# ForJadeForest/DistillCLIP

Measured on AMD Instinct MI355X. Metric: image-text pairs/sec (distill step), higher is better.
Workload: dtype bf16; 1 GPU; l_clip.yaml dual distill: ViT-B/32 CLIP teacher -> weight-shared ViT(6x768,24h,R2) + text(4x768,12h,R2) students, 224px/77tok, losses out_l1+out_cos+0.1*cos_diff, fwd+loss+bwd+AdamW; global_batch=512, batch_per_gpu=512, parallelism=dp1, gradient_exchange=none, negatives=local (reference training_step semantics), optimizer_in_step=True, teacher_residual=fp16, saved_gelu_derivative=u8 fixed point, clock_probe=True

## Files before the change

distillclip_amd/csrc/gemm.hip:

```cpp

#include "gemm_common.h"
#include <atomic>

using namespace dgemm;

namespace {

constexpr int TILE_BYTES = (BM / 16) * (BK / 32) * SUB;
constexpr int CLD = BN + 4;
constexpr int NT_LDS = (4 * TILE_BYTES > BM * CLD * 4) ? 4 * TILE_BYTES : BM * CLD * 4;


__device__ __forceinline__ void stage_operand(const bf16_t* __restrict__ G, int64_t ld, int row0, int rows_max,
                                              int k0, char* lds_tile, int wave, int lane) {
    const int L = lane * 16;
    const int X = swz(L);
    const int r = X >> 6, c = (X >> 4) & 3;
#pragma unroll
    for (int s = 0; s < 4; ++s) {
        const int sub = wave * 4 + s;
        const int rb = sub >> 1, kb = sub & 1;
        int row = row0 + rb * 16 + r;
        row = row < rows_max ? row : rows_max - 1;
        const bf16_t* src = G + (int64_t)row * ld + (k0 + kb * 32 + c * 8);
        __builtin_amdgcn_global_load_lds((gbl_void*)src, (lds_void*)(lds_tile + sub * SUB), 16, 0, 0);
    }
}

template <int ACT, int OUT>
__global__ __launch_bounds__(256) void gemm_nt_kernel(GemmNT p) {
    extern __shared__ __attribute__((aligned(16))) char smem[];
    const int tid = threadIdx.x, lane = tid & 63;
    const int wave = __builtin_amdgcn_readfirstlane(tid >> 6);
    const int wm = wave >> 1, wn = wave & 1;

    const int nwg = p.tiles_m * p.tiles_n;
    const int t = xcd_remap(blockIdx.x, nwg);
    const int tm = t / p.tiles_n, tn = t % p.tiles_n;
    const int m0 = tm * BM, n0 = tn * BN;

    char* As = smem;
    char* Bs = smem + 2 * TILE_BYTES;

    f32x4 acc[4][4];
#pragma unroll
    for (int i = 0; i < 4; ++i)
#pragma unroll
        for (int j = 0; j < 4; ++j) acc[i][j] = f32x4{0.f, 0.f, 0.f, 0.f};

    const int nk = p.K / BK;
    stage_operand(p.A, p.lda, m0, p.M, 0, As, wave, lane);
    stage_operand(p.B, p.ldb, n0, p.N, 0, Bs, wave, lane);

    const int fragoff = swz((lane & 15) * 64 + (lane >> 4) * 16);

    for (int kt = 0; kt < nk; ++kt) {
        __syncthreads();
        if (kt + 1 < nk) {
            const int nb = (kt + 1) & 1;
            stage_operand(p.A, p.lda, m0, p.M, (kt + 1) * BK, As + nb * TILE_BYTES, wave, lane);
            stage_operand(p.B, p.ldb, n0, p.N, (kt + 1) * BK, Bs + nb * TILE_BYTES, wave, lane);
        }
        const char* a_t = As + (kt & 1) * TILE_BYTES;
        const char* b_t = Bs + (kt & 1) * TILE_BYTES;
#pragma unroll
        for (int kb = 0; kb < 2; ++kb) {
            bf16x8 af[4], bfr[4];
#pragma unroll
            for (int i = 0; i < 4; ++i)
                af[i] = *(const bf16x8*)(a_t + ((wm * 4 + i) * 2 + kb) * SUB + fragoff);
#pragma unroll
            for (int j = 0; j < 4; ++j)
                bfr[j] = *(const bf16x8*)(b_t + ((wn * 4 + j) * 2 + kb) * SUB + fragoff);
#pragma unroll
            for (int i = 0; i < 4; ++i)
#pragma unroll
                for (int j = 0; j < 4; ++j)
                    acc[i][j] = __builtin_amdgcn_mfma_f32_16x16x32_bf16(af[i], bfr[j], acc[i][j], 0, 0, 0);
        }
    }

    __syncthreads();
    float* cs = (float*)smem;
#pragma unroll
    for (int i = 0; i < 4; ++i)
#pragma unroll
        for (int j = 0; j < 4; ++j)
#pragma unroll
            for (int r = 0; r < 4; ++r)
                cs[(wm * 64 + i * 16 + (lane >> 4) * 4 + r) * CLD + wn * 64 + j * 16 + (lane & 15)] = acc[i][j][r];
    __syncthreads();
    const int cc = (tid & 15) * 8;
    const int col = n0 + cc;
    const bool col_ok = col < p.N;
    float bias[8];
#pragma unroll
    for (int e = 0; e < 8; ++e) bias[e] = 0.f;
    if (p.bias && col_ok) {
        const float4 b0 = *(const float4*)(p.bias + col), b1 = *(const float4*)(p.bias + col + 4);
        bias[0] = b0.x; bias[1] = b0.y; bias[2] = b0.z; bias[3] = b0.w; bias[4] = b1.x; bias[5] = b1.y; bias[6] = b1.z; bias[7] = b1.w;
    }
    float csum[8];
#pragma unroll
    for (int e = 0; e < 8; ++e) csum[e] = 0.f;
#pragma unroll
    for (int it = 0; it < 8; ++it) {
        const int rl = (tid >> 4) + it * 16;
        const int row = m0 + rl;
        if (row >= p.M || !col_ok) break;
        float v[8];
        {
            const float4 c0 = *(const float4*)(cs + rl * CLD + cc), c1 = *(const float4*)(cs + rl * CLD + cc + 4);
            v[0] = c0.x; v[1] = c0.y; v[2] = c0.z; v[3] = c0.w; v[4] = c1.x; v[5] = c1.y; v[6] = c1.z; v[7] = c1.w;
        }
#pragma unroll
        for (int e = 0; e < 8; ++e) v[e] = v[e] * p.alpha + bias[e];
        if (p.row_group > 0) {
            const float* ra = p.rowadd + (int64_t)(row % p.row_group) * p.N + col;
            const float4 a0 = *(const float4*)ra, a1 = *(const float4*)(ra + 4);
            v[0] += a0.x; v[1] += a0.y; v[2] += a0.z; v[3] += a0.w; v[4] += a1.x; v[5] += a1.y; v[6] += a1.z; v[7] += a1.w;
        }
        const int64_t o = (int64_t)row * p.ldc + col;
        {
            EpiSide sd;
            epilogue_load_side<ACT, OUT>(p, o, (int64_t)row * p.ldr + col, sd);
            float zero[8] = {0.f, 0.f, 0.f, 0.f, 0.f, 0.f, 0.f, 0.f}, unused[8];
            GemmNT q = p;
            q.alpha = 1.f; q.row_group = 0; q.colsum = nullptr;
            epilogue_vec8<ACT, OUT, 0>(q, v, row, col, o, (int64_t)row * p.ldr + col, zero, unused, sd);
        }
#pragma unroll
        for (int e = 0; e < 8; ++e) csum[e] += v[e];
    }
    if (p.colsum) {
        __syncthreads();
#pragma unroll
        for (int e = 0; e < 8; ++e) cs[(tid >> 4) * CLD + cc + e] = csum[e];
        __syncthreads();
        if (tid < BN && n0 + tid < p.N) {
            float x = 0.f;
#pragma unroll
            for (int r = 0; r < 16; ++r) x += cs[r * CLD + tid];
            unsafeAtomicAdd(p.colsum + n0 + tid, x);
        }
    }
}

constexpr int HT = 16384;

__device__ __forceinline__ void stage_half_perm(const bf16_t* __restrict__ G, int64_t ld, int row0, int rows_max, int k0,
                                                char* buf, int wave, int lane) {
    const int L = lane * 16;
    const int X = swz(L);
    const int r = X >> 6, c = (X >> 4) & 3;
    const int j = wave & 3;
    int row = row0 + (wave >> 2) * 64 + (j >> 1) * 32 + (r >> 2) * 8 + (j & 1) * 4 + (r & 3);
    row = row < rows_max ? row : rows_max - 1;
    const bf16_t* src = G + (int64_t)row * ld + k0 + c * 8;
    __builtin_amdgcn_global_load_lds((gbl_void*)src, (lds_void*)(buf + (wave * 2 + 0) * SUB), 16, 0, 0);
    __builtin_amdgcn_global_load_lds((gbl_void*)(src + 32), (lds_void*)(buf + (wave * 2 + 1) * SUB), 16, 0, 0);
}

template <int RH>
__device__ __forceinline__ void stage_rowhalf(const bf16_t* __restrict__ G, int64_t ld, int m0, int rows_max, int k0,
                                              char* abase, int hta, int dn, int wave, int lane) {
    const int L = lane * 16;
    const int X = swz(L);
    const int r = X >> 6, c = (X >> 4) & 3;
    constexpr int AROWS = RH * 32;
    {
        const int wv = RH == 3 ? wave % 6 : wave;
        const int g = wv / RH, i = wv % RH + dn * RH;
        int row = m0 + g * AROWS + i * 16 + r;
        row = row < rows_max ? row : rows_max - 1;
        const bf16_t* src = G + (int64_t)row * ld + k0 + c * 8;
        char* dst = abase + g * hta + (i * 2) * SUB;
        __builtin_amdgcn_global_load_lds((gbl_void*)src, (lds_void*)dst, 16, 0, 0);
        __builtin_amdgcn_global_load_lds((gbl_void*)(src + 32), (lds_void*)(dst + SUB), 16, 0, 0);
    }
    if (RH == 5) {
        const int e = wave & 3, rbk = 8 + (e >> 1), kb = e & 1;
        const int g = rbk / RH, i = rbk % RH + dn * RH;
        int row = m0 + g * AROWS + i * 16 + r;
        row = row < rows_max ? row : rows_max - 1;
        const bf16_t* src = G + (int64_t)row * ld + k0 + kb * 32 + c * 8;
        __builtin_amdgcn_global_load_lds((gbl_void*)src, (lds_void*)(abase + g * hta + (i * 2 + kb) * SUB), 16, 0, 0);
    }
}


__device__ __forceinline__ float row16_sum(float x) {
    auto dpp = [](float v, auto ctrl) {
        return __builtin_bit_cast(float, __builtin_amdgcn_update_dpp(0, __builtin_bit_cast(int, v), decltype(ctrl)::value, 0xf, 0xf, false));
    };
    x += dpp(x, std::integral_constant<int, 0xB1>{});
    x += dpp(x, std::integral_constant<int, 0x4E>{});
    x += dpp(x, std::integral_constant<int, 0x141>{});
    x += dpp(x, std::integral_constant<int, 0x140>{});
    return x;
}

template <int ACT, int OUT, int MI>
__global__ __launch_bounds__(512) void gemm_nt256_kernel(GemmNT p) {
    extern __shared__ __attribute__((aligned(16))) char smem[];
    constexpr int RH = MI / 2;
    constexpr int AROWS = MI * 16;
    constexpr int HTA = AROWS * BK * 2;
    constexpr int PAR = 2 * HT + 2 * HTA;
    constexpr int BMT = 2 * AROWS;
    const int tid = threadIdx.x, lane = tid & 63;
    const int wave = __builtin_amdgcn_readfirstlane(tid >> 6);
    const int wr = wave >> 2, wc = wave & 3;

    const int nwg = p.tiles_m * p.tiles_n;
    const int nk = p.K / BK;
    const int nload = 4 * nk;
    int m0, n0;
    auto locate = [&](int tl) {
        const int t = xcd_remap(tl, nwg);
        int tm, tn;
        if (p.group_n >= p.tiles_n) { tm = t / p.tiles_n; tn = t % p.tiles_n; }
        else {
            const int per = p.tiles_m * p.group_n;
            const int gi = t / per, rem = t - gi * per;
            const int left = p.tiles_n - gi * p.group_n;
            const int gw = left < p.group_n ? left : p.group_n;
            tm = rem / gw; tn = gi * p.group_n + rem % gw;
        }
        m0 = tm * BMT; n0 = tn * 256;
    };
    locate(blockIdx.x);

    f32x4 acc[MI][4];

    const int ln = lane;
    auto issue = [&](int l) {
        const int tile = l >> 2, w = l & 3;
        char* par = smem + (tile & 1) * PAR;
        if (w < 2) stage_half_perm(p.B, p.ldb, n0 + w * 128, p.N, tile * BK, par + w * HT, wave, ln);
        else stage_rowhalf<RH>(p.A, p.lda, m0, p.M, tile * BK, par + 2 * HT, HTA, w - 2, wave, ln);
    };
    auto stamp = [&](int k) {
        if (p.stamps && tid == 0) {
            if (k == 3) WAIT_VMCNT(0);
            p.stamps[6 * (int64_t)blockIdx.x + k] = __builtin_readcyclecounter();
            if (k == 0) p.stamps[6 * (int64_t)blockIdx.x + 4] = __builtin_amdgcn_s_memrealtime();
            if (k == 3) p.stamps[6 * (int64_t)blockIdx.x + 5] = __builtin_amdgcn_s_memrealtime();
        }
    };
    stamp(0);
    if (p.clk && blockIdx.x == 0 && tid == 0) { p.clk[0] = __builtin_amdgcn_s_memtime(); p.clk[1] = __builtin_amdgcn_s_memrealtime(); }
#define WAIT_VM2(n8, n10) do { if (MI == 10) WAIT_VMCNT(n10); else WAIT_VMCNT(n8); } while (0)
    const int npro = nload < 7 ? nload : 7;
    for (int l = 0; l < npro; ++l) issue(l);
    const int a_off = 2 * HT + wr * HTA;
    const int b_off = (wc >> 1) * HT + (wc & 1) * 8 * SUB;
    const int fragoff = swz((ln & 15) * 64 + (ln >> 4) * 16);
#pragma unroll
    for (int i = 0; i < MI; ++i)
#pragma unroll
        for (int j = 0; j < 4; ++j) acc[i][j] = f32x4{0.f, 0.f, 0.f, 0.f};
    if (nload > 4) WAIT_VM2(8, 10); else WAIT_VMCNT(0);
    __builtin_amdgcn_s_barrier();
    stamp(1);
    if (wr == 1) __builtin_amdgcn_s_barrier();

    bf16x8 af[RH][2], b0[2][2], b1[2][2];

    for (int kt = 0; kt < nk; ++kt) {
        const char* base = smem + (kt & 1) * PAR;
        const char* ap = base + a_off + fragoff;
        const char* bp = base + b_off + fragoff;
#pragma unroll
        for (int j = 0; j < 2; ++j)
#pragma unroll
            for (int kb = 0; kb < 2; ++kb) {
                b0[j][kb] = *(const bf16x8*)(bp + (j * 2 + kb) * SUB);
                b1[j][kb] = *(const bf16x8*)(bp + ((2 + j) * 2 + kb) * SUB);
            }
        __builtin_amdgcn_sched_barrier(0);
#pragma unroll
        for (int i = 0; i < RH; ++i)
#pragma unroll
            for (int kb = 0; kb < 2; ++kb) af[i][kb] = *(const bf16x8*)(ap + (i * 2 + kb) * SUB);
        if (kt + 1 < nk) { issue(4 * (kt + 1) + 3); WAIT_VM2(8, 10); }
        else WAIT_VMCNT(0);
        WAIT_LGKM0();
        __builtin_amdgcn_s_barrier();
        __builtin_amdgcn_s_setprio(1);
#pragma unroll
        for (int kb = 0; kb < 2; ++kb)
#pragma unroll
            for (int i = 0; i < RH; ++i) {
#pragma unroll
                for (int j = 0; j < 2; ++j)
                    acc[i][j] = __builtin_amdgcn_mfma_f32_16x16x32_bf16(b0[j][kb], af[i][kb], acc[i][j], 0, 0, 0);
#pragma unroll
                for (int j = 0; j < 2; ++j)
                    acc[i][2 + j] = __builtin_amdgcn_mfma_f32_16x16x32_bf16(b1[j][kb], af[i][kb], acc[i][2 + j], 0, 0, 0);
            }
        __builtin_amdgcn_s_setprio(0);
        __builtin_amdgcn_s_barrier();
#pragma unroll
        for (int i = 0; i < RH; ++i)
#pragma unroll
            for (int kb = 0; kb < 2; ++kb) af[i][kb] = *(const bf16x8*)(ap + ((RH + i) * 2 + kb) * SUB);
        if (kt + 2 < nk) { issue(4 * (kt + 2)); issue(4 * (kt + 2) + 1); issue(4 * (kt + 2) + 2); WAIT_VM2(8, 10); }
        else if (kt + 1 < nk) WAIT_VM2(2, 3);
        else WAIT_VMCNT(0);
        WAIT_LGKM0();
        __builtin_amdgcn_s_barrier();
        __builtin_amdgcn_s_setprio(1);
#pragma unroll
        for (int kb = 0; kb < 2; ++kb)
#pragma unroll
            for (int i = 0; i < RH; ++i) {
#pragma unroll
                for (int j = 0; j < 2; ++j)
                    acc[RH + i][j] = __builtin_amdgcn_mfma_f32_16x16x32_bf16(b0[j][kb], af[i][kb], acc[RH + i][j], 0, 0, 0);
#pragma unroll
                for (int j = 0; j < 2; ++j)
                    acc[RH + i][2 + j] = __builtin_amdgcn_mfma_f32_16x16x32_bf16(b1[j][kb], af[i][kb], acc[RH + i][2 + j], 0, 0, 0);
            }
        __builtin_amdgcn_s_setprio(0);
        __builtin_amdgcn_s_barrier();
    }
    if (wr == 0) __builtin_amdgcn_s_barrier();
    stamp(2);
    const int m0c = m0, n0c = n0;
    const int g = ln >> 4, rl = ln & 15;

    const int colb = n0c + wc * 64 + g * 8;
    float bias[2][8], csum[2][8];
#pragma unroll
    for (int jp = 0; jp < 2; ++jp) {
#pragma unroll
        for (int e = 0; e < 8; ++e) { bias[jp][e] = 0.f; csum[jp][e] = 0.f; }
        const int col = colb + jp * 32;
        if (p.bias && col < p.N) {
            const float4 q0 = *(const float4*)(p.bias + col), q1 = *(const float4*)(p.bias + col + 4);
            bias[jp][0] = q0.x; bias[jp][1] = q0.y; bias[jp][2] = q0.z; bias[jp][3] = q0.w;
            bias[jp][4] = q1.x; bias[jp][5] = q1.y; bias[jp][6] = q1.z; bias[jp][7] = q1.w;
        }
    }
    constexpr bool OUT_F32 = OUT == 1;
    constexpr bool SIDE = OUT != 0 || ACT == 3 || ACT == 4;
    constexpr int NU = 2 * MI;
    constexpr int BU = !SIDE ? NU : (OUT_F32 ? ((ACT == 3 || ACT == 4) ? 4 : (MI == 8 ? 8 : (MI == 6 ? 6 : 5))) : (MI == 10 ? 10 : NU));
    static_assert(NU % BU == 0, "batch size must divide the unit count");
    EpiSide side[SIDE ? BU : 1];
    const int row0 = m0c + wr * AROWS + rl;
    const int64_t o0 = (int64_t)row0 * p.ldc + colb, r0off = (int64_t)row0 * p.ldr + colb;
    const int64_t ostep = 16 * p.ldc, rstep = 16 * p.ldr;
    const bool full = m0c + BMT <= p.M && n0c + 256 <= p.N;
    auto run_units = [&](auto mode_tag) {
        constexpr int MODE = decltype(mode_tag)::value;
#pragma unroll
        for (int ub = 0; ub < NU; ub += BU) {
            if (SIDE) {
#pragma unroll
                for (int u = ub; u < ub + BU; ++u) {
                    const int i = u >> 1, jp = u & 1;
                    if (full || (row0 + i * 16 < p.M && colb + jp * 32 < p.N))
                        epilogue_load_side<ACT, OUT>(p, o0 + i * ostep + jp * 32, r0off + i * rstep + jp * 32, side[u - ub]);
                }
            }
#pragma unroll
            for (int u = ub; u < ub + BU; ++u) {
                const int i = u >> 1, jp = u & 1;
                const int row = row0 + i * 16, col = colb + jp * 32;
                if (full || (row < p.M && col < p.N)) {
                    float v[8];
#pragma unroll
                    for (int r = 0; r < 4; ++r) { v[r] = acc[i][2 * jp][r]; v[4 + r] = acc[i][2 * jp + 1][r]; }
                    epilogue_vec8<ACT, OUT, MODE>(p, v, row, col, o0 + i * ostep + jp * 32, r0off + i * rstep + jp * 32, bias[jp], csum[jp],
                                                      side[SIDE ? u - ub : 0]);
                }
            }
        }
    };
    const bool lean = p.row_group == 0 && ((ACT == 5 || ACT == 6) ? p.aux_out != nullptr : p.aux_out == nullptr) && (OUT != 0 ? p.residual != nullptr : p.residual == nullptr);
    if constexpr (OUT != 0) {
        if (lean) run_units(std::integral_constant<int, 3>{});
        else run_units(std::integral_constant<int, 0>{});
    } else if constexpr (ACT == 3 || ACT == 4) {
        if (lean && p.colsum) run_units(std::integral_constant<int, 2>{});
        else run_units(std::integral_constant<int, 0>{});
    } else {
        if (lean && !p.colsum) run_units(std::integral_constant<int, 1>{});
        else if (lean) run_units(std::integral_constant<int, 2>{});
        else run_units(std::integral_constant<int, 0>{});
    }
    if (OUT == 0 && p.colsum) {
        float* cs = (float*)smem;
#pragma unroll
        for (int jp = 0; jp < 2; ++jp)
#pragma unroll
            for (int e = 0; e < 8; ++e) {
                const float x = row16_sum(csum[jp][e]);
                if (rl == 0) cs[wr * 256 + wc * 64 + jp * 32 + g * 8 + e] = x;
            }
        WAIT_LGKM0();
        __builtin_amdgcn_s_barrier();
        const int tc = wave * 64 + ln;
        if (tc < 256 && n0c + tc < p.N) unsafeAtomicAdd(p.colsum + n0c + tc, cs[tc] + cs[256 + tc]);
    }
    stamp(3);
    if (p.clk && blockIdx.x == 0 && tid == 0) { p.clk[2] = __builtin_amdgcn_s_memtime(); p.clk[3] = __builtin_amdgcn_s_memrealtime(); }
}

constexpr int TP = 128, TQ = 128, TC = 64;
constexpr int TROW = 288;
constexpr int TTILE = TC * TROW;

struct GemmTN {
    const bf16_t* A; int64_t lda;
    const bf16_t* B; int64_t ldb;
    float* out; int64_t ldo;
    int M, P, Q;
    int tiles_p, tiles_q, splits, chunk;
    unsigned long long* stamps;
    float* partial;
};

__device__ __forceinline__ void tn_load(const bf16_t* __restrict__ G, int64_t ld, int m0, int m_end, int c0, int cols,
                                        int tid, u32x4 (&regs)[4]) {
#pragma unroll
    for (int s = 0; s < 4; ++s) {
        const int idx = s * 256 + tid;
        const int r = idx >> 4, c = (idx & 15) * 8;
        const int row = m0 + r, col = c0 + c;
        if (row < m_end && col < cols) regs[s] = *(const u32x4*)(G + (int64_t)row * ld + col);
        else regs[s] = u32x4{0u, 0u, 0u, 0u};
    }
}
__device__ __forceinline__ void tn_store(char* tile, int tid, const u32x4 (&regs)[4]) {
#pragma unroll
    for (int s = 0; s < 4; ++s) {
        const int idx = s * 256 + tid;
        const int r = idx >> 4, c = (idx & 15);
        *(u32x4*)(tile + r * TROW + c * 16) = regs[s];
    }
}

typedef __attribute__((address_space(3))) s16x4 lds_s16x4;

__device__ __forceinline__ bf16x8 tr_frag(const char* tile, int r0, int x0, int lane) {
    const int g = lane >> 4, q = (lane >> 2) & 3, pp = lane & 3;
// ... 225 lines not shown
    const int tid = threadIdx.x, lane = tid & 63;
    const int wave = __builtin_amdgcn_readfirstlane(tid >> 6);
    const int wr = wave >> 2, wc = wave & 3;

    const int tiles = p.tiles_p * p.tiles_q;
    const int t = xcd_remap(blockIdx.x, tiles * p.splits);
    const int split = t / tiles, tile = t - split * tiles;
    const int tq = tile % p.tiles_q, tp = tile / p.tiles_q;
    const int p0 = tp * 256, q0 = tq * 256;
    const int m_begin = split * p.chunk;
    const int m_end = min(p.M, m_begin + p.chunk);
    if (m_begin >= m_end) return;
    const int nk = (m_end - m_begin) / TC;
    const int nload = 4 * nk;

    f32x4 acc[8][4];
#pragma unroll
    for (int i = 0; i < 8; ++i)
#pragma unroll
        for (int j = 0; j < 4; ++j) acc[i][j] = f32x4{0.f, 0.f, 0.f, 0.f};

    const char* srcs[4][2];
    tn_half_sources(p.B, p.ldb, m_begin, q0, wave, lane, srcs[0]);
    tn_half_sources(p.B, p.ldb, m_begin, q0 + 128, wave, lane, srcs[1]);
    tn_half_sources(p.A, p.lda, m_begin, p0, wave, lane, srcs[2]);
    tn_half_sources(p.A, p.lda, m_begin, p0 + 128, wave, lane, srcs[3]);
    const int64_t step_b = (int64_t)TC * p.ldb * 2, step_a = (int64_t)TC * p.lda * 2;
    auto issue = [&](int l) {
        const int kt = l >> 2, w = l & 3;
        char* buf = smem + ((kt & 1) * 4 + w) * HT;
        if (w == 0) stage_half_tn(srcs[0], kt * step_b, buf, wave);
        else if (w == 1) stage_half_tn(srcs[1], kt * step_b, buf, wave);
        else if (w == 2) stage_half_tn(srcs[2], kt * step_a, buf, wave);
        else stage_half_tn(srcs[3], kt * step_a, buf, wave);
    };
    auto stamp = [&](int k) {
        if (p.stamps && tid == 0) {
            if (k == 3) WAIT_VMCNT(0);
            p.stamps[6 * (int64_t)blockIdx.x + k] = __builtin_readcyclecounter();
            if (k == 0) p.stamps[6 * (int64_t)blockIdx.x + 4] = __builtin_amdgcn_s_memrealtime();
            if (k == 3) p.stamps[6 * (int64_t)blockIdx.x + 5] = __builtin_amdgcn_s_memrealtime();
        }
    };
    stamp(0);
    const int npro = nload < 6 ? nload : 6;
#pragma unroll
    for (int l = 0; l < 6; ++l)
        if (l < npro) issue(l);
    if (nload > 4) WAIT_VMCNT(4); else WAIT_VMCNT(0);
    __builtin_amdgcn_s_barrier();
    stamp(1);
    if (wr == 1) __builtin_amdgcn_s_barrier();

    const int a_off = (2 + wr) * HT;
    const int b_off = (wc >> 1) * HT;
    const int bcol = (wc & 1) * 64;
    bf16x8 af[4][2], b0[2][2], b1[2][2];

    for (int kt = 0; kt < nk; ++kt) {
        const char* base = smem + (kt & 1) * 4 * HT;
        const char* at = base + a_off;
        const char* bt = base + b_off;
        const int k4 = kt * 4;
#pragma unroll
        for (int j = 0; j < 2; ++j) {
            const unsigned a0 = tr_frag_base(bt, bcol + j * 16, lane), a1 = tr_frag_base(bt, bcol + (2 + j) * 16, lane);
            b0[j][0] = tr_frag_asm<0>(a0); b0[j][1] = tr_frag_asm<32 * 256>(a0);
            b1[j][0] = tr_frag_asm<0>(a1); b1[j][1] = tr_frag_asm<32 * 256>(a1);
        }
        __builtin_amdgcn_sched_barrier(0);
#pragma unroll
        for (int i = 0; i < 4; ++i) {
            const unsigned a0 = tr_frag_base(at, i * 16, lane);
            af[i][0] = tr_frag_asm<0>(a0); af[i][1] = tr_frag_asm<32 * 256>(a0);
        }
        if (k4 + 6 < nload) issue(k4 + 6);
        if (k4 + 7 < nload) issue(k4 + 7);
        WAIT_LGKM0();
        __builtin_amdgcn_sched_barrier(0);
        __builtin_amdgcn_s_barrier();
        __builtin_amdgcn_s_setprio(1);
#pragma unroll
        for (int kb = 0; kb < 2; ++kb)
#pragma unroll
            for (int i = 0; i < 4; ++i) {
#pragma unroll
                for (int j = 0; j < 2; ++j)
                    acc[i][j] = __builtin_amdgcn_mfma_f32_16x16x32_bf16(af[i][kb], b0[j][kb], acc[i][j], 0, 0, 0);
#pragma unroll
                for (int j = 0; j < 2; ++j)
                    acc[i][2 + j] = __builtin_amdgcn_mfma_f32_16x16x32_bf16(af[i][kb], b1[j][kb], acc[i][2 + j], 0, 0, 0);
            }
        __builtin_amdgcn_s_setprio(0);
        __builtin_amdgcn_s_barrier();
        __builtin_amdgcn_sched_barrier(0);
#pragma unroll
        for (int i = 0; i < 4; ++i) {
            const unsigned a0 = tr_frag_base(at, (4 + i) * 16, lane);
            af[i][0] = tr_frag_asm<0>(a0); af[i][1] = tr_frag_asm<32 * 256>(a0);
        }
        if (k4 + 8 < nload) { issue(k4 + 8); issue(k4 + 9); WAIT_VMCNT(4); }
        else WAIT_VMCNT(0);
        WAIT_LGKM0();
        __builtin_amdgcn_sched_barrier(0);
        __builtin_amdgcn_s_barrier();
        __builtin_amdgcn_s_setprio(1);
#pragma unroll
        for (int kb = 0; kb < 2; ++kb)
#pragma unroll
            for (int i = 0; i < 4; ++i) {
#pragma unroll
                for (int j = 0; j < 2; ++j)
                    acc[4 + i][j] = __builtin_amdgcn_mfma_f32_16x16x32_bf16(af[i][kb], b0[j][kb], acc[4 + i][j], 0, 0, 0);
#pragma unroll
                for (int j = 0; j < 2; ++j)
                    acc[4 + i][2 + j] = __builtin_amdgcn_mfma_f32_16x16x32_bf16(af[i][kb], b1[j][kb], acc[4 + i][2 + j], 0, 0, 0);
            }
        __builtin_amdgcn_s_setprio(0);
        __builtin_amdgcn_s_barrier();
    }
    if (wr == 0) __builtin_amdgcn_s_barrier();
    stamp(2);

    float* cs = (float*)smem;
    constexpr int CL = 256 + 4;
#pragma unroll
    for (int q = 0; q < 4; ++q) {
        __syncthreads();
#pragma unroll
        for (int i = 0; i < 2; ++i)
#pragma unroll
            for (int j = 0; j < 4; ++j)
#pragma unroll
                for (int r = 0; r < 4; ++r)
                    cs[(wr * 32 + i * 16 + (lane >> 4) * 4 + r) * CL + wc * 64 + j * 16 + (lane & 15)] = acc[q * 2 + i][j][r];
        __syncthreads();
        if (p.partial) {
            float* dst = p.partial + ((int64_t)split * tiles + tile) * 65536;
#pragma unroll 4
            for (int it = 0; it < 8; ++it) {
                const int sl = (tid >> 6) + it * 8;
                const int rt = (sl >> 5) * 128 + q * 32 + (sl & 31);
                *(float4*)(dst + rt * 256 + (tid & 63) * 4) = *(const float4*)&cs[sl * CL + (tid & 63) * 4];
            }
        } else {
#pragma unroll 4
            for (int it = 0; it < 32; ++it) {
                const int sl = (tid >> 8) + it * 2;
                const int row = p0 + (sl >> 5) * 128 + q * 32 + (sl & 31);
                const int col = q0 + (tid & 255);
                unsafeAtomicAdd(p.out + (int64_t)row * p.ldo + col, cs[sl * CL + (tid & 255)]);
            }
        }
    }
    stamp(3);
}

__global__ __launch_bounds__(256) void tn256_reduce_kernel(const float* __restrict__ partial, int splits, int tiles, int tiles_q,
                                                           float* __restrict__ out, int64_t ldo) {
    const int idx = blockIdx.x * 256 + threadIdx.x;
    const int tile = idx >> 14, rt = (idx >> 6) & 255, c4 = idx & 63;
    if (tile >= tiles) return;
    const float* src = partial + (int64_t)tile * 65536 + rt * 256 + c4 * 4;
    float4 a = *(const float4*)src;
    for (int s = 1; s < splits; ++s) {
        const float4 v = *(const float4*)(src + (int64_t)s * tiles * 65536);
        a.x += v.x; a.y += v.y; a.z += v.z; a.w += v.w;
    }
    float* o = out + (int64_t)((tile / tiles_q) * 256 + rt) * ldo + (tile % tiles_q) * 256 + c4 * 4;
    float4 cur = *(const float4*)o;
    cur.x += a.x; cur.y += a.y; cur.z += a.z; cur.w += a.w;
    *(float4*)o = cur;
}

__global__ __launch_bounds__(256) void colsum_kernel(const bf16_t* __restrict__ X, int64_t ld, float* __restrict__ db,
                                                     int M, int N, int rows_per_block) {
    const int col = blockIdx.x * 256 + threadIdx.x;
    if (col >= N) return;
    const int r0 = blockIdx.y * rows_per_block;
    const int r1 = min(M, r0 + rows_per_block);
    float s0 = 0.f, s1 = 0.f, s2 = 0.f, s3 = 0.f;
    int r = r0;
    for (; r + 3 < r1; r += 4) {
        s0 += bf2f(X[(int64_t)r * ld + col]);
        s1 += bf2f(X[(int64_t)(r + 1) * ld + col]);
        s2 += bf2f(X[(int64_t)(r + 2) * ld + col]);
        s3 += bf2f(X[(int64_t)(r + 3) * ld + col]);
    }
    for (; r < r1; ++r) s0 += bf2f(X[(int64_t)r * ld + col]);
    unsafeAtomicAdd(db + col, (s0 + s1) + (s2 + s3));
}

__global__ __launch_bounds__(256) void colsum8_kernel(const bf16_t* __restrict__ X, int64_t ld, float* __restrict__ db,
                                                      int M, int N, int rows_per_block) {
    __shared__ float red[8][256 + 8];
    const int cg = threadIdx.x & 31, rl = threadIdx.x >> 5;
    const int col = blockIdx.x * 256 + cg * 8;
    const int r0 = blockIdx.y * rows_per_block;
    const int r1 = min(M, r0 + rows_per_block);
    float acc[8];
#pragma unroll
    for (int e = 0; e < 8; ++e) acc[e] = 0.f;
    if (col < N) {
        int r = r0 + rl;
        for (; r + 24 < r1; r += 32) {
            bf16x8 v[4];
#pragma unroll
            for (int u = 0; u < 4; ++u) v[u] = *(const bf16x8*)(X + (int64_t)(r + 8 * u) * ld + col);
#pragma unroll
            for (int u = 0; u < 4; ++u)
#pragma unroll
                for (int e = 0; e < 8; ++e) acc[e] += bf2f(v[u][e]);
        }
        for (; r < r1; r += 8) {
            const bf16x8 v = *(const bf16x8*)(X + (int64_t)r * ld + col);
#pragma unroll
            for (int e = 0; e < 8; ++e) acc[e] += bf2f(v[e]);
        }
    }
#pragma unroll
    for (int e = 0; e < 8; ++e) red[rl][cg * 8 + e] = acc[e];
    __syncthreads();
    const int c = blockIdx.x * 256 + threadIdx.x;
    if (c < N) {
        float x = 0.f;
#pragma unroll
        for (int w = 0; w < 8; ++w) x += red[w][threadIdx.x];
        unsafeAtomicAdd(db + c, x);
    }
}

bool use_256(const GemmNT& p) {
    static const int mode = [] { const char* e = getenv("DCLIP_GEMM256"); return e ? atoi(e) : 1; }();
    return mode != 0 && p.M >= 1024 && p.N >= 256;
}

std::atomic<unsigned long long*> g_clock_buf{nullptr};
std::atomic<long long> g_clock_cap{0};
std::atomic<long long> g_clock_count{0};
inline unsigned long long* next_clock_slot() {
    unsigned long long* buf = g_clock_buf.load(std::memory_order_acquire);
    const long long cap = g_clock_cap.load(std::memory_order_relaxed);
    if (!buf || cap <= 0) return nullptr;
    return buf + 4 * (g_clock_count.fetch_add(1, std::memory_order_relaxed) % cap);
}

template <int ACT>
int launch_nt(GemmNT p, int out, hipStream_t st) {
    if constexpr (ACT != 0) { if (out == 2) { dclip_set_error("dclip_gemm_nt: f16 output needs act = DCLIP_ACT_NONE"); return DCLIP_EINVAL; } }
    const bool out_f32 = out == 1;
    if (use_256(p) && !(out != 0 && p.colsum) && (ACT == 0 || out == 0)) {
        int tm = (p.M + 255) / 256;
        const int tn = (p.N + 255) / 256;
        static const int mode320 = [] { const char* e = getenv("DCLIP_GEMM320"); return e ? atoi(e) : 1; }();
        int mi = 8;
        if (mode320) {
            const double nkt = (double)(p.K / BK), e8 = out_f32 ? 40000.0 : out == 2 ? 24000.0 : (ACT == 0 || ACT == 4 ? 9500.0 : 14000.0);
            auto cost = [&](int rows, double per_kt, double escale) {
                const int tmx = (p.M + rows - 1) / rows;
                return (double)((tmx * tn + 255) / 256) * (3300.0 + nkt * per_kt + escale * e8);
            };
            const double c8 = cost(256, 2750.0, 1.0), c10 = cost(320, 3200.0, 1.25), c6 = cost(192, 2150.0, 0.75);
            if (mode320 == 2) mi = 10;
            else if (mode320 == 6) mi = 6;
            else {
                if (c10 < c8) mi = 10;
                if (c6 < (mi == 10 ? c10 : c8) * 0.97) mi = 6;
            }
            tm = (p.M + mi * 32 - 1) / (mi * 32);
        }
        p.tiles_m = tm; p.tiles_n = tn;
        p.clk = next_clock_slot();
        const int ntiles = p.tiles_m * p.tiles_n;
        {
            const double panel = 512.0 * (double)p.K, a_bytes = 2.0 * (double)p.M * (double)p.K;
            double best = 0.0; int best_g = tn;
            for (int g = 1; g <= tn; ++g) {
                const int ngroups = (tn + g - 1) / g;
                const double b_term = (g * panel <= 2.5e6) ? 8.0 * g * panel * (ngroups > 8 ? ngroups / 8.0 : 1.0)
                                                           : (double)ntiles / 32.0 * g * panel;
                const double cost = a_bytes * ngroups + b_term;
                if (g == 1 || cost < best * 0.999) { best = cost; best_g = g; }
            }
            p.group_n = best_g;
        }
        if (mi == 10) {
            const size_t lds320 = 2 * (2 * HT + 2 * 160 * BK * 2) + 16;
            if (out_f32) { if constexpr (ACT == 0) hipLaunchKernelGGL((gemm_nt256_kernel<0, 1, 10>), dim3(ntiles), dim3(512), lds320, st, p); }
            else if (out == 2) { if constexpr (ACT == 0) hipLaunchKernelGGL((gemm_nt256_kernel<0, 2, 10>), dim3(ntiles), dim3(512), lds320, st, p); }
            else hipLaunchKernelGGL((gemm_nt256_kernel<ACT, 0, 10>), dim3(ntiles), dim3(512), lds320, st, p);
            return dclip_check_launch("dclip_gemm_nt");
        }
        if (mi == 6) {
            const size_t lds192 = 2 * (2 * HT + 2 * 96 * BK * 2) + 16;
            if (out_f32) { if constexpr (ACT == 0) hipLaunchKernelGGL((gemm_nt256_kernel<0, 1, 6>), dim3(ntiles), dim3(512), lds192, st, p); }
            else if (out == 2) { if constexpr (ACT == 0) hipLaunchKernelGGL((gemm_nt256_kernel<0, 2, 6>), dim3(ntiles), dim3(512), lds192, st, p); }
            else hipLaunchKernelGGL((gemm_nt256_kernel<ACT, 0, 6>), dim3(ntiles), dim3(512), lds192, st, p);
            return dclip_check_launch("dclip_gemm_nt");
        }
        const size_t lds256 = 8 * HT + 16;
        if (out_f32) { if constexpr (ACT == 0) hipLaunchKernelGGL((gemm_nt256_kernel<0, 1, 8>), dim3(ntiles), dim3(512), lds256, st, p); }
        else if (out == 2) { if constexpr (ACT == 0) hipLaunchKernelGGL((gemm_nt256_kernel<0, 2, 8>), dim3(ntiles), dim3(512), lds256, st, p); }
        else hipLaunchKernelGGL((gemm_nt256_kernel<ACT, 0, 8>), dim3(ntiles), dim3(512), lds256, st, p);
        return dclip_check_launch("dclip_gemm_nt");
    }
    const int grid = p.tiles_m * p.tiles_n;
    const size_t lds = NT_LDS;
    if (out_f32) hipLaunchKernelGGL((gemm_nt_kernel<ACT, 1>), dim3(grid), dim3(256), lds, st, p);
    else if (out == 2) { if constexpr (ACT == 0) hipLaunchKernelGGL((gemm_nt_kernel<0, 2>), dim3(grid), dim3(256), lds, st, p); }
    else hipLaunchKernelGGL((gemm_nt_kernel<ACT, 0>), dim3(grid), dim3(256), lds, st, p);
    return dclip_check_launch("dclip_gemm_nt");
}

unsigned long long* g_gemm_stamps = nullptr;
std::atomic<long long> g_tn_atomic_fallbacks{0};

}

extern "C" int dclip_trace_gemm_stamps(void* buf) { g_gemm_stamps = (unsigned long long*)buf; return 0; }
extern "C" int64_t dclip_trace_gemm_clock(void* buf, int64_t cap) {
    const long long n = g_clock_count.exchange(0, std::memory_order_relaxed);
    g_clock_cap.store(buf ? (long long)cap : 0, std::memory_order_relaxed);
    g_clock_buf.store((unsigned long long*)buf, std::memory_order_release);
    return (int64_t)n;
}
extern "C" int64_t dclip_gemm_tn_atomic_fallbacks(void) { return (int64_t)g_tn_atomic_fallbacks.load(std::memory_order_relaxed); }

extern "C" int dclip_gemm_nt(const void* A, int64_t lda, const void* B, int64_t ldb, void* C, int64_t ldc,
                             int64_t M, int64_t N, int64_t K, float alpha, const float* bias, int act,
                             const void* aux_in, void* aux_out, const void* residual, int64_t ldr, int out_dtype,
                             int64_t row_group, const float* rowadd, float* colsum_acc, void* stream) {
    DCLIP_REQUIRE(A && B && C, "dclip_gemm_nt: null operand");
    DCLIP_REQUIRE(M > 0 && N > 0 && K > 0, "dclip_gemm_nt: empty problem M=%ld N=%ld K=%ld", (long)M, (long)N, (long)K);
    DCLIP_REQUIRE(K % BK == 0, "dclip_gemm_nt: K=%ld must be a multiple of %d", (long)K, BK);
    DCLIP_REQUIRE(lda % 8 == 0 && ldb % 8 == 0 && ((uintptr_t)A % 16) == 0 && ((uintptr_t)B % 16) == 0,
                  "dclip_gemm_nt: operand rows must be 16-byte aligned (lda=%ld ldb=%ld)", (long)lda, (long)ldb);
    DCLIP_REQUIRE(N % 8 == 0 && ldc % 8 == 0 && ((uintptr_t)C % 16) == 0, "dclip_gemm_nt: N and ldc must be multiples of 8 and C 16-byte aligned (N=%ld ldc=%ld)", (long)N, (long)ldc);
    DCLIP_REQUIRE(out_dtype >= 0 && out_dtype <= 2, "dclip_gemm_nt: bad output dtype %d (0 bf16, 1 f32, 2 f16)", out_dtype);
    DCLIP_REQUIRE(!residual || (ldr % (out_dtype == 2 ? 8 : 4) == 0 && ((uintptr_t)residual % 16) == 0), "dclip_gemm_nt: residual rows must be 16-byte aligned");
    DCLIP_REQUIRE(act >= 0 && act <= 6, "dclip_gemm_nt: bad activation code %d", act);
    DCLIP_REQUIRE(out_dtype != 2 || act == 0, "dclip_gemm_nt: f16 output needs act = DCLIP_ACT_NONE");
    DCLIP_REQUIRE((act != DCLIP_ACT_DGELU && act != DCLIP_ACT_MULAUX) || aux_in, "dclip_gemm_nt: DGELU / MULAUX need aux_in");
    DCLIP_REQUIRE(!aux_in || ((uintptr_t)aux_in % 16) == 0, "dclip_gemm_nt: aux_in must be 16-byte aligned");
    DCLIP_REQUIRE(!aux_out || ((uintptr_t)aux_out % 16) == 0, "dclip_gemm_nt: aux_out must be 16-byte aligned");
    DCLIP_REQUIRE(row_group == 0 || rowadd, "dclip_gemm_nt: row_group needs rowadd");
    DCLIP_REQUIRE(M < (1LL << 31) && N < (1LL << 31), "dclip_gemm_nt: dimension overflow");
    GemmNT p;
    p.A = (const bf16_t*)A; p.lda = lda; p.B = (const bf16_t*)B; p.ldb = ldb; p.C = C; p.ldc = ldc;
    p.M = (int)M; p.N = (int)N; p.K = (int)K; p.alpha = alpha; p.bias = bias;
    p.aux_in = aux_in; p.aux_out = aux_out; p.residual = residual; p.ldr = ldr;
    p.row_group = (int)row_group; p.rowadd = rowadd; p.colsum = colsum_acc;
    p.tiles_m = (int)((M + BM - 1) / BM); p.tiles_n = (int)((N + BN - 1) / BN);
    p.stamps = g_gemm_stamps;
    p.group_n = 1 << 30;
    p.clk = nullptr;
    hipStream_t st = (hipStream_t)stream;
    const int out_f32 = out_dtype == 1;
    const double aux_b = (act == DCLIP_ACT_MULAUX || act == DCLIP_ACT_GELU_SAVE || act == DCLIP_ACT_QUICKGELU_SAVE) ? 1.0 : 2.0;
    TraceScope tr(DCLIP_TRACE_GEMM_NT, 2.0 * (double)M * (double)N * (double)K,
                  2.0 * ((double)M * K + (double)N * K) + ((out_f32 ? 4.0 : 2.0) + (residual ? (out_dtype == 2 ? 2.0 : 4.0) : 0.0) + (aux_in ? aux_b : 0.0) + (aux_out ? aux_b : 0.0)) * (double)M * N,
                  stream, (int)M, (int)N, (int)K,
                  act + 8 * (out_f32 != 0) + 16 * (residual != nullptr) + 32 * (colsum_acc != nullptr) + 64 * (out_dtype == 2));
    switch (act) {
        case 0: return launch_nt<0>(p, out_dtype, st);
        case 1: return launch_nt<1>(p, out_dtype, st);
        case 2: return launch_nt<2>(p, out_dtype, st);
        case 3: return launch_nt<3>(p, out_dtype, st);
        case 4: return launch_nt<4>(p, out_dtype, st);
        case 5: return launch_nt<5>(p, out_dtype, st);
        default: return launch_nt<6>(p, out_dtype, st);
    }
}

extern "C" size_t dclip_gemm_tn_workspace_bytes(void) { return (size_t)384 * 65536 * sizeof(float); }

extern "C" int dclip_gemm_tn_acc(const void* A, int64_t lda, const void* B, int64_t ldb, float* dW, int64_t ldo,
                                 int64_t M, int64_t P, int64_t Q, int splits, void* workspace, size_t ws_bytes, void* stream) {
    DCLIP_REQUIRE(A && B && dW, "dclip_gemm_tn_acc: null operand");
    DCLIP_REQUIRE(M > 0 && P > 0 && Q > 0, "dclip_gemm_tn_acc: empty problem");
    DCLIP_REQUIRE(P % 8 == 0 && Q % 8 == 0 && lda % 8 == 0 && ldb % 8 == 0 &&
                  ((uintptr_t)A % 16) == 0 && ((uintptr_t)B % 16) == 0,
                  "dclip_gemm_tn_acc: P, Q, lda, ldb must be multiples of 8 and bases 16-byte aligned");
    DCLIP_REQUIRE(splits >= 1, "dclip_gemm_tn_acc: splits must be >= 1");
    GemmTN p;
    p.A = (const bf16_t*)A; p.lda = lda; p.B = (const bf16_t*)B; p.ldb = ldb; p.out = dW; p.ldo = ldo;
    p.M = (int)M; p.P = (int)P; p.Q = (int)Q; p.stamps = g_gemm_stamps; p.partial = nullptr;
    p.tiles_p = (int)((P + TP - 1) / TP); p.tiles_q = (int)((Q + TQ - 1) / TQ);
    int chunk = (int)((M + splits - 1) / splits);
    chunk = ((chunk + TC - 1) / TC) * TC;
    p.chunk = chunk;
    p.splits = (int)((M + chunk - 1) / chunk);
    const int grid = p.tiles_p * p.tiles_q * p.splits;
    const bool fast = M % TC == 0 && P >= 8 && Q >= 8;
    if (fast && P % 256 == 0 && Q % 256 == 0 && (P / 256) * (Q / 256) >= 16 && M >= 4096) {
        GemmTN q = p;
        q.tiles_p = (int)(P / 256); q.tiles_q = (int)(Q / 256);
        const int tiles = q.tiles_p * q.tiles_q;
        int s = (256 + tiles / 2) / tiles;
        if (s < 1) s = 1;
        int ch = (int)((M + s - 1) / s);
        ch = ((ch + TC - 1) / TC) * TC;
        q.chunk = ch;
        q.splits = (int)((M + ch - 1) / ch);
        TraceScope tr2(DCLIP_TRACE_GEMM_TN, 2.0 * (double)M * (double)P * (double)Q, 2.0 * ((double)M * P + (double)M * Q) + 4.0 * (double)P * Q, stream, (int)M, (int)P, (int)Q, 256);
        static const int tn_partial = [] { const char* e = getenv("DCLIP_TN_PARTIAL"); return e ? atoi(e) : 1; }();
        const size_t need = (size_t)tiles * q.splits * 65536 * sizeof(float);
        const bool part = tn_partial != 0 && workspace && ws_bytes >= need && ldo % 4 == 0 && ((uintptr_t)dW % 16) == 0 && q.splits > 1;
        if (!part && q.splits > 1) g_tn_atomic_fallbacks.fetch_add(1, std::memory_order_relaxed);
        q.partial = part ? (float*)workspace : nullptr;
        hipLaunchKernelGGL(gemm_tn256_kernel, dim3(tiles * q.splits), dim3(512), 8 * HT, (hipStream_t)stream, q);
        if (part)
            hipLaunchKernelGGL(tn256_reduce_kernel, dim3((unsigned)(tiles * 64)), dim3(256), 0, (hipStream_t)stream, (const float*)workspace,
                               q.splits, tiles, q.tiles_q, dW, ldo);
        return dclip_check_launch("dclip_gemm_tn_acc");
    }
    TraceScope tr(DCLIP_TRACE_GEMM_TN, 2.0 * (double)M * (double)P * (double)Q, 2.0 * ((double)M * P + (double)M * Q) + 4.0 * (double)P * Q, stream, (int)M, (int)P, (int)Q, 128);
    if (fast) hipLaunchKernelGGL(gemm_tn_glds_kernel, dim3(grid), dim3(256), TN_LDS, (hipStream_t)stream, p);
    else hipLaunchKernelGGL(gemm_tn_kernel, dim3(grid), dim3(256), 4 * TTILE, (hipStream_t)stream, p);
    return dclip_check_launch("dclip_gemm_tn_acc");
}

extern "C" int dclip_colsum_acc(const void* X, int64_t ld, float* db, int64_t M, int64_t N, void* stream) {
    DCLIP_REQUIRE(X && db && M > 0 && N > 0, "dclip_colsum_acc: bad argument");
    const int colblocks = (int)((N + 255) / 256);
    int rows_per_block = (int)((M * colblocks + 511) / 512);
    rows_per_block = rows_per_block < 16 ? 16 : (rows_per_block > 512 ? 512 : (rows_per_block + 3) & ~3);
    dim3 grid((unsigned)((N + 255) / 256), (unsigned)((M + rows_per_block - 1) / rows_per_block));
    if (N % 8 == 0 && ld % 8 == 0 && ((uintptr_t)X & 15) == 0)
        hipLaunchKernelGGL(colsum8_kernel, grid, dim3(256), 0, (hipStream_t)stream, (const bf16_t*)X, ld, db, (int)M, (int)N,
                           rows_per_block);
    else
        hipLaunchKernelGGL(colsum_kernel, grid, dim3(256), 0, (hipStream_t)stream, (const bf16_t*)X, ld, db, (int)M, (int)N,
                           rows_per_block);
    return dclip_check_launch("dclip_colsum_acc");
}
```

Before: 18910 pairs/s.

## Add 64-row GEMM kernel with 4-deep LDS ring for small grids

Adds a small-grid NT GEMM path that halves the M tile to 64 rows, doubling the workgroup count for GEMMs with fewer than 128 tiles. It also replaces double buffering with a 4-stage ring that waits on vmcnt instead of issuing full barriers. The epilogue is factored into a shared helper. The aim is better CU occupancy on small problems at the cost of less reuse of the B operand per tile.

```diff
diff --git a/distillclip_amd/csrc/gemm.hip b/distillclip_amd/csrc/gemm.hip
--- a/distillclip_amd/csrc/gemm.hip
+++ b/distillclip_amd/csrc/gemm.hip
@@ -27,69 +27,8 @@
     }
 }
 
-template <int ACT, int OUT>
-__global__ __launch_bounds__(256) void gemm_nt_kernel(GemmNT p) {
-    extern __shared__ __attribute__((aligned(16))) char smem[];
-    const int tid = threadIdx.x, lane = tid & 63;
-    const int wave = __builtin_amdgcn_readfirstlane(tid >> 6);
-    const int wm = wave >> 1, wn = wave & 1;
-
-    const int nwg = p.tiles_m * p.tiles_n;
-    const int t = xcd_remap(blockIdx.x, nwg);
-    const int tm = t / p.tiles_n, tn = t % p.tiles_n;
-    const int m0 = tm * BM, n0 = tn * BN;
-
-    char* As = smem;
-    char* Bs = smem + 2 * TILE_BYTES;
-
-    f32x4 acc[4][4];
-#pragma unroll
-    for (int i = 0; i < 4; ++i)
-#pragma unroll
-        for (int j = 0; j < 4; ++j) acc[i][j] = f32x4{0.f, 0.f, 0.f, 0.f};
-
-    const int nk = p.K / BK;
-    stage_operand(p.A, p.lda, m0, p.M, 0, As, wave, lane);
-    stage_operand(p.B, p.ldb, n0, p.N, 0, Bs, wave, lane);
-
-    const int fragoff = swz((lane & 15) * 64 + (lane >> 4) * 16);
-
-    for (int kt = 0; kt < nk; ++kt) {
-        __syncthreads();
-        if (kt + 1 < nk) {
-            const int nb = (kt + 1) & 1;
-            stage_operand(p.A, p.lda, m0, p.M, (kt + 1) * BK, As + nb * TILE_BYTES, wave, lane);
-            stage_operand(p.B, p.ldb, n0, p.N, (kt + 1) * BK, Bs + nb * TILE_BYTES, wave, lane);
-        }
-        const char* a_t = As + (kt & 1) * TILE_BYTES;
-        const char* b_t = Bs + (kt & 1) * TILE_BYTES;
-#pragma unroll
-        for (int kb = 0; kb < 2; ++kb) {
-            bf16x8 af[4], bfr[4];
-#pragma unroll
-            for (int i = 0; i < 4; ++i)
-                af[i] = *(const bf16x8*)(a_t + ((wm * 4 + i) * 2 + kb) * SUB + fragoff);
-#pragma unroll
-            for (int j = 0; j < 4; ++j)
-                bfr[j] = *(const bf16x8*)(b_t + ((wn * 4 + j) * 2 + kb) * SUB + fragoff);
-#pragma unroll
-            for (int i = 0; i < 4; ++i)
-#pragma unroll
-                for (int j = 0; j < 4; ++j)
-                    acc[i][j] = __builtin_amdgcn_mfma_f32_16x16x32_bf16(af[i], bfr[j], acc[i][j], 0, 0, 0);
-        }
-    }
-
-    __syncthreads();
-    float* cs = (float*)smem;
-#pragma unroll
-    for (int i = 0; i < 4; ++i)
-#pragma unroll
-        for (int j = 0; j < 4; ++j)
-#pragma unroll
-            for (int r = 0; r < 4; ++r)
-                cs[(wm * 64 + i * 16 + (lane >> 4) * 4 + r) * CLD + wn * 64 + j * 16 + (lane & 15)] = acc[i][j][r];
-    __syncthreads();
+template <int ACT, int OUT, int ROWS>
+__device__ __forceinline__ void epilogue_from_lds(const GemmNT& p, float* cs, int m0, int n0, int tid) {
     const int cc = (tid & 15) * 8;
     const int col = n0 + cc;
     const bool col_ok = col < p.N;
@@ -104,7 +43,7 @@
 #pragma unroll
     for (int e = 0; e < 8; ++e) csum[e] = 0.f;
 #pragma unroll
-    for (int it = 0; it < 8; ++it) {
+    for (int it = 0; it < ROWS / 16; ++it) {
         const int rl = (tid >> 4) + it * 16;
         const int row = m0 + rl;
         if (row >= p.M || !col_ok) break;
@@ -144,6 +83,160 @@
             unsafeAtomicAdd(p.colsum + n0 + tid, x);
         }
     }
+}
+
+template <int ACT, int OUT>
+__global__ __launch_bounds__(256) void gemm_nt_kernel(GemmNT p) {
+    extern __shared__ __attribute__((aligned(16))) char smem[];
+    const int tid = threadIdx.x, lane = tid & 63;
+    const int wave = __builtin_amdgcn_readfirstlane(tid >> 6);
+    const int wm = wave >> 1, wn = wave & 1;
+
+    const int nwg = p.tiles_m * p.tiles_n;
+    const int t = xcd_remap(blockIdx.x, nwg);
+    const int tm = t / p.tiles_n, tn = t % p.tiles_n;
+    const int m0 = tm * BM, n0 = tn * BN;
+
+    char* As = smem;
+    char* Bs = smem + 2 * TILE_BYTES;
+
+    f32x4 acc[4][4];
+#pragma unroll
+    for (int i = 0; i < 4; ++i)
+#pragma unroll
+        for (int j = 0; j < 4; ++j) acc[i][j] = f32x4{0.f, 0.f, 0.f, 0.f};
+
+    const int nk = p.K / BK;
+    stage_operand(p.A, p.lda, m0, p.M, 0, As, wave, lane);
+    stage_operand(p.B, p.ldb, n0, p.N, 0, Bs, wave, lane);
+
+    const int fragoff = swz((lane & 15) * 64 + (lane >> 4) * 16);
+
+    for (int kt = 0; kt < nk; ++kt) {
+        __syncthreads();
+        if (kt + 1 < nk) {
+            const int nb = (kt + 1) & 1;
+            stage_operand(p.A, p.lda, m0, p.M, (kt + 1) * BK, As + nb * TILE_BYTES, wave, lane);
+            stage_operand(p.B, p.ldb, n0, p.N, (kt + 1) * BK, Bs + nb * TILE_BYTES, wave, lane);
+        }
+        const char* a_t = As + (kt & 1) * TILE_BYTES;
+        const char* b_t = Bs + (kt & 1) * TILE_BYTES;
+#pragma unroll
+        for (int kb = 0; kb < 2; ++kb) {
+            bf16x8 af[4], bfr[4];
+#pragma unroll
+            for (int i = 0; i < 4; ++i)
+                af[i] = *(const bf16x8*)(a_t + ((wm * 4 + i) * 2 + kb) * SUB + fragoff);
+#pragma unroll
+            for (int j = 0; j < 4; ++j)
+                bfr[j] = *(const bf16x8*)(b_t + ((wn * 4 + j) * 2 + kb) * SUB + fragoff);
+#pragma unroll
+            for (int i = 0; i < 4; ++i)
+#pragma unroll
+                for (int j = 0; j < 4; ++j)
+                    acc[i][j] = __builtin_amdgcn_mfma_f32_16x16x32_bf16(af[i], bfr[j], acc[i][j], 0, 0, 0);
+        }
+    }
+
+    __syncthreads();
+    float* cs = (float*)smem;
+#pragma unroll
+    for (int i = 0; i < 4; ++i)
+#pragma unroll
+        for (int j = 0; j < 4; ++j)
+#pragma unroll
+            for (int r = 0; r < 4; ++r)
+                cs[(wm * 64 + i * 16 + (lane >> 4) * 4 + r) * CLD + wn * 64 + j * 16 + (lane & 15)] = acc[i][j][r];
+    __syncthreads();
+    epilogue_from_lds<ACT, OUT, BM>(p, cs, m0, n0, tid);
+}
+
+constexpr int SG_BM = 64;
+constexpr int SG_ABYTES = (SG_BM / 16) * (BK / 32) * SUB;
+constexpr int SG_STAGE = SG_ABYTES + TILE_BYTES;
+constexpr int SG_DEPTH = 4;
+constexpr int SG_LDS = SG_DEPTH * SG_STAGE;
+constexpr int SG_MAX_TILES = 128;
+static_assert(SG_LDS >= SG_BM * CLD * 4, "the staged C tile fits the ring");
+
+__device__ __forceinline__ void sg_stage(const GemmNT& p, int m0, int n0, int k0, char* st, int wave, int lane) {
+    const int X = swz(lane * 16);
+    const int r = X >> 6, c = (X >> 4) & 3;
+#pragma unroll
+    for (int s = 0; s < 2; ++s) {
+        const int sub = wave * 2 + s;
+        const int rb = sub >> 1, kb = sub & 1;
+        int row = m0 + rb * 16 + r;
+        row = row < p.M ? row : p.M - 1;
+        const bf16_t* src = p.A + (int64_t)row * p.lda + (k0 + kb * 32 + c * 8);
+        __builtin_amdgcn_global_load_lds((gbl_void*)src, (lds_void*)(st + sub * SUB), 16, 0, 0);
+    }
+    stage_operand(p.B, p.ldb, n0, p.N, k0, st + SG_ABYTES, wave, lane);
+}
+
+template <int ACT, int OUT>
+__global__ __launch_bounds__(256) void gemm_nt_small_kernel(GemmNT p) {
+    extern __shared__ __attribute__((aligned(16))) char smem[];
+    const int tid = threadIdx.x, lane = tid & 63;
+    const int wave = __builtin_amdgcn_readfirstlane(tid >> 6);
+    const int wm = wave >> 1, wn = wave & 1;
+
+    const int nwg = p.tiles_m * p.tiles_n;
+    const int t = xcd_remap(blockIdx.x, nwg);
+    const int tm = t / p.tiles_n, tn = t % p.tiles_n;
+    const int m0 = tm * SG_BM, n0 = tn * BN;
+
+    f32x4 acc[2][4];
+#pragma unroll
+    for (int i = 0; i < 2; ++i)
+#pragma unroll
+        for (int j = 0; j < 4; ++j) acc[i][j] = f32x4{0.f, 0.f, 0.f, 0.f};
+
+    const int nk = p.K / BK;
+#pragma unroll
+    for (int s = 0; s < SG_DEPTH - 1; ++s)
+        if (s < nk) sg_stage(p, m0, n0, s * BK, smem + s * SG_STAGE, wave, lane);
+
+    const int fragoff = swz((lane & 15) * 64 + (lane >> 4) * 16);
+
+    for (int kt = 0; kt < nk; ++kt) {
+        const int younger = (nk - 1 < kt + 2 ? nk - 1 : kt + 2) - kt;
+        if (younger == 2) WAIT_VMCNT(12);
+        else if (younger == 1) WAIT_VMCNT(6);
+        else WAIT_VMCNT(0);
+        __builtin_amdgcn_s_barrier();
+        if (kt + SG_DEPTH - 1 < nk)
+            sg_stage(p, m0, n0, (kt + SG_DEPTH - 1) * BK, smem + ((kt + SG_DEPTH - 1) % SG_DEPTH) * SG_STAGE, wave, lane);
+        const char* a_t = smem + (kt % SG_DEPTH) * SG_STAGE;
+        const char* b_t = a_t + SG_ABYTES;
+#pragma unroll
+        for (int kb = 0; kb < 2; ++kb) {
+            bf16x8 af[2], bfr[4];
+#pragma unroll
+            for (int i = 0; i < 2; ++i)
+                af[i] = *(const bf16x8*)(a_t + ((wm * 2 + i) * 2 + kb) * SUB + fragoff);
+#pragma unroll
+            for (int j = 0; j < 4; ++j)
+                bfr[j] = *(const bf16x8*)(b_t + ((wn * 4 + j) * 2 + kb) * SUB + fragoff);
+#pragma unroll
+            for (int i = 0; i < 2; ++i)
+#pragma unroll
+                for (int j = 0; j < 4; ++j)
+                    acc[i][j] = __builtin_amdgcn_mfma_f32_16x16x32_bf16(af[i], bfr[j], acc[i][j], 0, 0, 0);
+        }
+    }
+
+    __syncthreads();
+    float* cs = (float*)smem;
+#pragma unroll
+    for (int i = 0; i < 2; ++i)
+#pragma unroll
+        for (int j = 0; j < 4; ++j)
+#pragma unroll
+            for (int r = 0; r < 4; ++r)
+                cs[(wm * 32 + i * 16 + (lane >> 4) * 4 + r) * CLD + wn * 64 + j * 16 + (lane & 15)] = acc[i][j][r];
+    __syncthreads();
+    epilogue_from_lds<ACT, OUT, SG_BM>(p, cs, m0, n0, tid);
 }
 
 constexpr int HT = 16384;
@@ -975,6 +1068,15 @@
         if (out_f32) { if constexpr (ACT == 0) hipLaunchKernelGGL((gemm_nt256_kernel<0, 1, 8>), dim3(ntiles), dim3(512), lds256, st, p); }
         else if (out == 2) { if constexpr (ACT == 0) hipLaunchKernelGGL((gemm_nt256_kernel<0, 2, 8>), dim3(ntiles), dim3(512), lds256, st, p); }
         else hipLaunchKernelGGL((gemm_nt256_kernel<ACT, 0, 8>), dim3(ntiles), dim3(512), lds256, st, p);
+        return dclip_check_launch("dclip_gemm_nt");
+    }
+    static const int smallgrid = [] { const char* e = getenv("DCLIP_GEMM_SMALLGRID"); return e ? atoi(e) : 1; }();
+    if (smallgrid != 0 && p.tiles_m * p.tiles_n < SG_MAX_TILES) {
+        p.tiles_m = (p.M + SG_BM - 1) / SG_BM;
+        const int sgrid = p.tiles_m * p.tiles_n;
+        if (out_f32) hipLaunchKernelGGL((gemm_nt_small_kernel<ACT, 1>), dim3(sgrid), dim3(256), SG_LDS, st, p);
+        else if (out == 2) { if constexpr (ACT == 0) hipLaunchKernelGGL((gemm_nt_small_kernel<0, 2>), dim3(sgrid), dim3(256), SG_LDS, st, p); }
+        else hipLaunchKernelGGL((gemm_nt_small_kernel<ACT, 0>), dim3(sgrid), dim3(256), SG_LDS, st, p);
         return dclip_check_launch("dclip_gemm_nt");
     }
     const int grid = p.tiles_m * p.tiles_n;
```

Result: no change. 18890 pairs/s (-0.1%).
